# samyak0210/ViNet

Hardware: AMD Instinct MI355X
Metric: clips/sec training (32x224x384 bf16) (higher is better)
Workload: dtype bf16; 1 GPU; ViNet DHF1K training, 32x224x384 bf16, 192 clip(s)/GPU/step, kldiv + fused Adam, 1xMI355X; global_batch=192, local_batch=192, parallelism=dp1

## Files before the change

### include/vinet_hip.h

```cpp
#ifndef VINET_HIP_H
#define VINET_HIP_H

#include <stddef.h>
#include <stdint.h>

#ifdef __cplusplus
extern "C" {
#endif

#define VINET_ABI_VERSION 16

enum { VINET_F32 = 0, VINET_BF16 = 1,
       VINET_F32S = 2 };
enum { VINET_ACT_NONE = 0, VINET_ACT_RELU = 1, VINET_ACT_SIGMOID = 2 };
enum { VINET_CONV_GENERIC = 0, VINET_CONV_STEM = 1 };

typedef struct VinetTensor {
  void* ptr;
  int32_t B, T, H, W, C;
  int32_t ld;
  int64_t sB;
} VinetTensor;

typedef struct VinetAffine {
// ... 115 lines not shown
int vinet_channel_sum(const VinetTensor* x, int32_t dtype, float* workspace, int32_t Cout, float* out,
                      int32_t accumulate, void* stream);

typedef struct VinetPoolDesc {
  int32_t dtype;
  int32_t kT, kH, kW, sT, sH, sW, pT, pH, pW;
} VinetPoolDesc;
int vinet_maxpool3d(const VinetPoolDesc* d, const VinetTensor* x, VinetAffine pre, const VinetTensor* y,
                    uint8_t* argmax, void* stream);
int vinet_maxpool3d_bwd(const VinetPoolDesc* d, const VinetTensor* dy, const uint8_t* argmax, const VinetTensor* dx,
                        int32_t accumulate, void* stream);
int vinet_maxpool3d_kernel_name(const VinetPoolDesc* d, const VinetTensor* x, VinetAffine pre, const VinetTensor* y,
                                const uint8_t* argmax, char* buf, int32_t n);
int vinet_maxpool3d_bwd_kernel_name(const VinetPoolDesc* d, const VinetTensor* dy, const uint8_t* argmax,
                                    const VinetTensor* dx, char* buf, int32_t n);
int vinet_bn_bwd_pool_ok(const VinetPoolDesc* pool, const VinetTensor* z, const VinetTensor* dp, const VinetTensor* dx, int32_t dtype);
int vinet_bn_bwd_reduce_pool(const VinetPoolDesc* pool, const VinetTensor* dp, const uint8_t* argmax, const VinetTensor* gacc,
                             int32_t accumulate, const VinetTensor* z, int32_t dtype, VinetAffine fwd, const float* mean,
                             const float* invstd, float* partials, void* stream);
int vinet_bn_bwd_apply_pool(const VinetPoolDesc* pool, const VinetTensor* dp, const uint8_t* argmax, const VinetTensor* gacc,
                            int32_t accumulate, const VinetTensor* z, int32_t dtype, VinetAffine fwd, const float* mean,
                            const float* invstd, const float* c1, const float* c2, const VinetTensor* dx, void* stream);

int vinet_upsample2x(const VinetTensor* x, const VinetTensor* y, int32_t dtype, void* stream);
int vinet_upsample2x_bwd(const VinetTensor* dy, const VinetTensor* dx, int32_t dtype, int32_t accumulate, void* stream);
int vinet_upsample2x_bwd_relu(const VinetTensor* dy, const VinetTensor* dx, const VinetTensor* xf, int32_t dtype, void* stream);

int vinet_unfold1d(const VinetTensor* x, const VinetTensor* y, int32_t dtype, int32_t stride, int32_t pad, void* stream);

int vinet_loss_fwd(int32_t which, const float* s, const void* gt, int32_t gt_is_f64, int32_t B, int32_t n,
// ... 105 lines not shown
```

### vinet_amd/_lib.py

```python
import ctypes as C
import os

HERE = os.path.dirname(os.path.abspath(__file__))
LIB_PATH = os.environ.get("VINET_LIB") or os.path.join(HERE, "libvinet_hip.so")

F32, BF16 = 0, 1
F32S = 2
ACT_NONE, ACT_RELU, ACT_SIGMOID = 0, 1, 2
CONV_GENERIC, CONV_STEM = 0, 1
ABI_VERSION = 16


class CTensor(C.Structure):
    _fields_ = [("ptr", C.c_void_p), ("B", C.c_int32), ("T", C.c_int32), ("H", C.c_int32), ("W", C.c_int32),
                ("C", C.c_int32), ("ld", C.c_int32), ("sB", C.c_int64)]


class CAffine(C.Structure):
    _fields_ = [("scale", C.c_void_p), ("shift", C.c_void_p), ("relu", C.c_int32)]


class CConvDesc(C.Structure):
    _fields_ = [("dtype", C.c_int32), ("out_dtype", C.c_int32), ("mode", C.c_int32), ("x", CTensor), ("y", CTensor),
                ("oT", C.c_int32), ("oH", C.c_int32), ("oW", C.c_int32),
# ... 60 lines not shown
    "vinet_bn_bwd_reduce": [_PT, _PT, _i32, CAffine, _vp, _vp, _vp, _vp],
    "vinet_conv3d_wgrad_fuses_bn_bwd": [_PW],
    "vinet_conv3d_fuses_dgrad_phases": [_PC],
    "vinet_conv3d_bn_bwd_stats_rows": [_PC],
    "vinet_bn_partials_fold": [_vp, _i32, _i32, _vp, _i32, _vp],
    "vinet_bn_bwd_finalize": [_vp, _i32, _i32, _i32, _f64, _vp, _i32, _vp, _vp, _vp, _vp, _vp, _vp],
    "vinet_bn_bwd_apply": [_PT, _PT, _i32, CAffine, _vp, _vp, _vp, _vp, _PT, _vp],
    "vinet_bn_bwd_apply_split": [_PT, _PT, CAffine, _vp, _vp, _vp, _vp, _PT, _PT, _PT, _vp],
    "vinet_bn_bwd_pool_ok": [_PP, _PT, _PT, _PT, _i32],
    "vinet_bn_bwd_reduce_pool": [_PP, _PT, _vp, _PT, _i32, _PT, _i32, CAffine, _vp, _vp, _vp, _vp],
    "vinet_bn_bwd_apply_pool": [_PP, _PT, _vp, _PT, _i32, _PT, _i32, CAffine, _vp, _vp, _vp, _vp, _PT, _vp],
    "vinet_act_bwd": [_PT, _i32, _PT, _i32, _i32, _PT, _i32, _vp],
    "vinet_channel_sum": [_PT, _i32, _vp, _i32, _vp, _i32, _vp],
    "vinet_maxpool3d": [_PP, _PT, CAffine, _PT, _vp, _vp],
    "vinet_maxpool3d_bwd": [_PP, _PT, _vp, _PT, _i32, _vp],
    "vinet_maxpool3d_kernel_name": [_PP, _PT, CAffine, _PT, _vp, C.c_char_p, _i32],
    "vinet_maxpool3d_bwd_kernel_name": [_PP, _PT, _vp, _PT, C.c_char_p, _i32],
    "vinet_upsample2x": [_PT, _PT, _i32, _vp],
    "vinet_unfold1d": [_PT, _PT, _i32, _i32, _i32, _vp],
    "vinet_upsample2x_bwd": [_PT, _PT, _i32, _i32, _vp],
    "vinet_upsample2x_bwd_relu": [_PT, _PT, _PT, _i32, _vp],
    "vinet_loss_fwd": [_i32, _vp, _vp, _i32, _i32, _i32, _vp, _vp, _vp],
    "vinet_loss_bwd": [_i32, _vp, _vp, _i32, _i32, _i32, _vp, _vp, _f32, _i32, _vp, _vp],
    "vinet_auc_judd_workspace": [_i32, _i32],
    "vinet_auc_judd": [_vp, _i32, _vp, _i32, _i32, _i32, _i32, _vp, C.c_size_t, _vp, _vp, _vp, _vp],
    "vinet_auc_shuffled_workspace": [_i32, _i32, _i32, _f64],
    "vinet_auc_shuffled": [_vp, _i32, _vp, _i32, _vp, _i32, _i64, _i32, _i32, _i32, _f64, _i64, _vp, _vp, _i32, _vp, C.c_size_t,
                           _vp, _vp, _vp, _vp, _vp],
    "vinet_auc_borji_workspace": [_i32, _i32, _i32, _f64],
    "vinet_auc_borji": [_vp, _i32, _vp, _i32, _i32, _i32, _i32, _f64, _i64, _vp, _vp, _i32, _vp, C.c_size_t, _vp, _vp, _vp, _vp],
# ... 104 lines not shown
```

### vinet_amd/csrc/pool.hip

```cpp
#include "pool_gather.h"

struct PoolP { int kT, kH, kW, sT, sH, sW, pT, pH, pW; FastDiv dsT, dsH, dsW; };
static inline PoolP make_poolp(const VinetPoolDesc* d) {
  PoolP p = {d->kT, d->kH, d->kW, d->sT, d->sH, d->sW, d->pT, d->pH, d->pW, make_fastdiv((uint32_t)d->sT), make_fastdiv((uint32_t)d->sH), make_fastdiv((uint32_t)d->sW)};
  return p;
}

template <typename T> VN_DEV float pool_round(float v) { return v; }
template <> VN_DEV float pool_round<bf16_t>(float v) { return bf2f(f2bf(v)); }
template <typename T> VN_DEV float4 pool_pre4(float4 v, const Affine& pre, int c) {
  v = affine4(v, pre, c);
  if (pre.scale) { v.x = pool_round<T>(v.x); v.y = pool_round<T>(v.y); v.z = pool_round<T>(v.z); v.w = pool_round<T>(v.w); }
  return v;
}
template <typename T> VN_DEV float pool_pre(float f, float sc, float sh, const Affine& pre) {
  float v = fmaf(f, sc, sh);
  if (pre.relu) v = fmaxf(v, 0.f);
  if (pre.scale) v = pool_round<T>(v);
  return v;
}
VN_DEV void pool_column(const TView& v, uint32_t col, int& b, int& h, int& w) {
  const uint32_t r1 = fdiv(col, v.dW);
  w = (int)(col - r1 * (uint32_t)v.W);
  const uint32_t r2 = fdiv(r1, v.dH);
// ... 311 lines not shown
      *(unsigned long long*)(argmax + ovox * y.C + c0) = oi;
    }
  }
}


VN_DEV uint32_t pool_code2(uint32_t u) {
  const uint32_t m = ((u >> 15) & 0x00010001u) * 0x7fffu;
  return u ^ (m | 0x80008000u);
}
VN_DEV uint32_t pool_decode2(uint32_t k) {
  const uint32_t m = (((k >> 15) & 0x00010001u) ^ 0x00010001u) * 0x7fffu;
  return k ^ (m | 0x80008000u);
}

__global__ __launch_bounds__(256) void maxpool_fwd8_pk_kernel(PoolP p, TView x, Affine pre, TView y, uint8_t* __restrict__ argmax, long total) {
  const long i = (long)blockIdx.x * blockDim.x + threadIdx.x;
  if (i >= total) return;
  const int G = y.C >> 3;
  const uint32_t vox_u = (uint32_t)(i / G);
  const int g = (int)(i - (long)vox_u * G);
  int b, to, ho, wo;
  decode_vox(y, (long)vox_u, b, to, ho, wo);
  f32x2_v sc2[4], sh2[4];
  const bool aff = pre.scale != nullptr;
#pragma unroll
  for (int e = 0; e < 4; ++e) {
    sc2[e] = aff ? (f32x2_v){pre.scale[g * 8 + 2 * e], pre.scale[g * 8 + 2 * e + 1]} : (f32x2_v){1.f, 1.f};
    sh2[e] = aff ? (f32x2_v){pre.shift[g * 8 + 2 * e], pre.shift[g * 8 + 2 * e + 1]} : (f32x2_v){0.f, 0.f};
  }
  uint32_t best[8];
// ... 13 lines not shown
        uint32_t w4[4] = {q.x, q.y, q.z, q.w};
        const uint32_t ck = last - (uint32_t)((kt * p.kH + kh) * p.kW + kw);
#pragma unroll
        for (int e = 0; e < 4; ++e) {
          if (aff) {
            if (pre.relu) w4[e] = pre_relu_pair(w4[e], sc2[e], sh2[e]);
            else w4[e] = pack2bf(fmaf(__uint_as_float(w4[e] << 16), sc2[e].x, sh2[e].x), fmaf(__uint_as_float(w4[e] & 0xffff0000u), sc2[e].y, sh2[e].y));
          } else if (pre.relu) {
            asm("v_pk_max_i16 %0, %1, 0" : "=v"(w4[e]) : "v"(w4[e]));
          }
          const uint32_t c = pool_code2(w4[e]);
          const uint32_t klo = (c << 16) | ck, khi = (c & 0xffff0000u) | ck;
          best[2 * e] = best[2 * e] > klo ? best[2 * e] : klo;
          best[2 * e + 1] = best[2 * e + 1] > khi ? best[2 * e + 1] : khi;
        }
      }
    }
  }
  uint32_t ov[4];
  unsigned long long bi = 0;
#pragma unroll
  for (int e = 0; e < 8; ++e) {
    const uint32_t k = best[e];
    if (e & 1) ov[e >> 1] |= k & 0xffff0000u; else ov[e >> 1] = k >> 16;
    bi |= (unsigned long long)(last - (k & 0xffu)) << (8 * e);
  }
  uint4 o;
  o.x = pool_decode2(ov[0]); o.y = pool_decode2(ov[1]); o.z = pool_decode2(ov[2]); o.w = pool_decode2(ov[3]);
  *(uint4*)((bf16_t*)y.p + vox_off(y, b, to, ho, wo) + g * 8) = o;
  if (argmax) *(unsigned long long*)(argmax + (long)vox_u * y.C + g * 8) = bi;
}

__global__ __launch_bounds__(512) void maxpool_k3s1_pk_kernel(TView x, Affine pre, TView y, uint8_t* __restrict__ argmax,
                                                              int tilesH, int tilesW) {
  __shared__ __attribute__((aligned(16))) uint16_t P[2][100][64];
  __shared__ __attribute__((aligned(16))) float S[2][64];
  const int tid = threadIdx.x;
  const int oct = tid & 7, pos = tid >> 3;
  const int ph = pos >> 3, pw = pos & 7;
  int bid = blockIdx.x;
  const int ncg = (x.C + 63) >> 6;
  const int cg = bid % ncg; bid /= ncg;
  const int tw = bid % tilesW; bid /= tilesW;
  const int th = bid % tilesH; bid /= tilesH;
  const int b = bid;
// ... 572 lines not shown
                                                 r.tilesH, r.tilesW);) break;
    case POOL_TSLIDE8:
      DISPATCH_T(d->dtype, T, hipLaunchKernelGGL(maxpool_tslide8_kernel<T>, grid, lanes, 0, s, p, xv, a, yv, argmax, r.n);) break;
    case POOL_TSLIDE:
      DISPATCH_T(d->dtype, T, hipLaunchKernelGGL(maxpool_tslide_kernel<T>, grid, lanes, 0, s, p, xv, a, yv, argmax, r.n);) break;
    case POOL_FWD8_PK: hipLaunchKernelGGL(maxpool_fwd8_pk_kernel, grid, lanes, 0, s, p, xv, a, yv, argmax, r.n); break;
    case POOL_FWD8:
      DISPATCH_T(d->dtype, T, hipLaunchKernelGGL(maxpool_fwd8_kernel<T>, grid, lanes, 0, s, p, xv, a, yv, argmax, r.n);) break;
    case POOL_FWD:
      DISPATCH_T(d->dtype, T, hipLaunchKernelGGL(maxpool_fwd_kernel<T>, grid, lanes, 0, s, p, xv, a, yv, argmax, r.n);) break;
    default: break;
  }
  return vn_launch_status(r.name);
}

extern "C" int vinet_maxpool3d_bwd(const VinetPoolDesc* d, const VinetTensor* dy, const uint8_t* argmax,
                                   const VinetTensor* dx, int32_t accumulate, void* stream) {
  if (pool_bwd_args(d, dy, argmax, dx)) return -1;
  const PoolRoute r = pool_bwd_route(d, dy, argmax, dx);
  const PoolP p = make_poolp(d);
  const TView gv = make_view(*dy), xv = make_view(*dx);
  const hipStream_t s = (hipStream_t)stream;
  const dim3 lanes(256), grid(ew_grid(r.n));
  switch (r.kind) {
    case POOL_BWD_K3S1_TW3: hipLaunchKernelGGL(maxpool_bwd_k3s1_tw3_kernel, grid, lanes, 0, s, gv, argmax, xv, accumulate, r.n); break;
    case POOL_BWD_K3S1_TWALK:
      DISPATCH_T(d->dtype, T, hipLaunchKernelGGL(maxpool_bwd_k3s1_twalk_kernel<T>, grid, lanes, 0, s, gv, argmax, xv, accumulate, r.n);) break;
    case POOL_BWD_K3S1:
      DISPATCH_T(d->dtype, T, hipLaunchKernelGGL(maxpool_bwd_k3s1_kernel<T>, grid, lanes, 0, s, gv, argmax, xv, accumulate, r.n);) break;
    case POOL_BWD_K133S2:
// ... 14 lines not shown
```

### vinet_amd/engine.py

```python
import ctypes as C
import itertools
import math
import os
import weakref

import torch

from . import _lib as L

F32, BF16 = L.F32, L.BF16
F32S = L.F32S
TORCH_DT = {F32: torch.float32, BF16: torch.bfloat16}
ESIZE = {F32: 4, BF16: 2}
EG = {F32: 4, BF16: 8}

_DEFAULT_DTYPE = BF16
_WEIGHTS_EPOCH = 0
_UNPACK_TABLES = {}
_SIDE_STREAMS = {}

_CONFIG = dict(
    WGRAD_SIDE_STREAM=True,
    WGRAD_CUS=208,
    WGRAD_CUS_DEC=208,
# ... 10 lines not shown
    BRANCH_STREAMS_BWD_MIN_BATCH=8,
    BRANCH_STREAMS_SWAP=True,
    STEM_FOLD=True,
    JOINT_ENTRY=1,
    BN_BWD_FUSE=1,
    SHARE_SKIP_GRAD=True,
    DEFER_DECODER_WGRAD=1,
    DEFER_DECODER_WGRAD_F32S=0,
    PERSISTENT_DW=1,
    MATERIALIZE_NT=800,
    SPLIT_WGRAD_BF16=1,
    SPLIT_IN_APPLY=1,
    DGRAD_BN_STATS=1,
    UPSAMPLE_BWD_RELU=1,
    POOL_BWD_IN_BN=1,
    PARAM_GRAD_MODE="fused",
    DBG_SPIN_SIDE=0,
    DBG_SPIN_MAIN=0,
    DBG_SPIN_FORK=0,
    ABLATE="",
)
globals().update(_CONFIG)
_ABLATE, _ABLATE_TAGS = set(), []


def configure(**kw):
    global _ABLATE, _ABLATE_TAGS
    old = {}
    for k, v in kw.items():
        K = k.upper()
# ... 140 lines not shown
        n = self.nvox * self.C
        assert n % 4 == 0
        return View(self.buf, self.off, 1, 1, 1, n // 4, 4, 4, n, self.dt)

    def torch5(self):
        return torch.as_strided(self.buf, (self.B, self.T, self.H, self.W, self.C),
                                (self.sB, self.H * self.W * self.ld, self.W * self.ld, self.ld, 1), self.off)

    def same_dims(self, o):
        return (self.B, self.T, self.H, self.W, self.C) == (o.B, o.T, o.H, o.W, o.C)


class Act:
    __slots__ = ("v", "scale", "shift", "relu", "_grad", "grad_ready", "needs_grad", "parent", "pc0", "pt0", "fold",
                 "indep", "ready_of", "grad_marks", "mean", "invstd", "alias_of", "n_readers", "act_out", "grad_masked", "prows", "bn1",
                 "pool_rec")

    def __init__(self, v, scale=None, shift=None, relu=False, needs_grad=False, mean=None, invstd=None):
        self.v, self.scale, self.shift, self.relu = v, scale, shift, relu
        self.mean, self.invstd = mean, invstd
        self._grad, self.grad_ready, self.needs_grad = None, False, needs_grad
        self.parent, self.pc0, self.pt0 = None, 0, 0
        self.fold = None
        self.indep = False
        self.ready_of = None
        self.grad_marks = 0
        self.alias_of = None
        self.n_readers = 0
        self.act_out = 0
        self.grad_masked = -1
        self.prows = None
        self.bn1 = False
        self.pool_rec = None

    @property
    def plain(self):
        return self.scale is None and not self.relu

    def affine(self):
        return L.CAffine(_ptr(self.scale), _ptr(self.shift), 1 if self.relu else 0)

    def sub_chan(self, c0, c1):
        a = Act(self.v.chan(c0, c1), None if self.scale is None else self.scale[c0:c1],
                None if self.shift is None else self.shift[c0:c1], self.relu, self.needs_grad,
                None if self.mean is None else self.mean[c0:c1], None if self.invstd is None else self.invstd[c0:c1])
        a.parent, a.pc0, a.pt0 = self, c0, None
        return a

# ... 314 lines not shown
    g = a.grad_view()
    B, Cc, T, H, W = gt.shape
    sb, sc, st, sh, sw = gt.stride()
    ctx.call("vinet_import_ncdhw", gt.data_ptr(), sb, sc, st, sh, sw, Cc, C.byref(g.ct()), g.dt, ctx.stream)
    a.mark_grad_ready()


def materialize(ctx, a, dst=None, out_dt=None, share_grad=False):
    v = a.v
    alias = dst is None and (out_dt is None or out_dt == v.dt) and v.dt == ctx.dt
    if dst is None:
        dt = ctx.dt if out_dt is None else out_dt
        dst = Act(View.alloc(v.B, v.T, v.H, v.W, v.C, dt, v.device))
    out = dst.v
    assert out.same_dims(v) and dst.plain
    ctx.call("vinet_copy_affine", C.byref(v.ct()), v.dt, a.affine(), C.byref(out.ct()), out.dt, 0, ctx.stream)
    dst.needs_grad = a.needs_grad
    if alias:
        dst.parent, dst.pc0, dst.pt0 = a, 0, None
        dst.alias_of = a
        return dst
    _note_reader(ctx, a)
    if (share_grad and SHARE_SKIP_GRAD and ctx.recording and a.needs_grad and a.parent is None and a._grad is None
            and dst.parent is not None and out.dt == v.dt):
        a.parent, a.pc0, a.pt0 = dst, 0, None
        return dst
    if ctx.recording and a.needs_grad:
        def bwd():
            dg = dst.grad_view()
            tg = a.grad_view()
            ctx.call("vinet_copy_affine", C.byref(dg.ct()), dg.dt, L.CAffine(None, None, 0), C.byref(tg.ct()), tg.dt,
                     1 if a.is_grad_ready() else 0, ctx.stream)
            a.mark_grad_ready()
        ctx.record(bwd)
    return dst


def new_concat(ctx, B, T, H, W, Ctot, pending):
    v = View.alloc(B, T, H, W, Ctot, ctx.dt, ctx.device)
    if pending:
        st = ctx.training
        return Act(v, ctx.f32(Ctot), ctx.f32(Ctot), relu=True, needs_grad=True, mean=ctx.f32(Ctot) if st else None,
                   invstd=ctx.f32(Ctot) if st else None)
    return Act(v, needs_grad=True)



def _phase_taps_1d(I, O, k, s, p):
    out = []
    for r in range(s):
# ... 781 lines not shown
                and dx.same_dims(bx.v) and x.root().grad_marks + 1 == x.root().n_readers)
    part = None
    for ph in phases:
        d = _conv_desc(ctx, L.CONV_GENERIC, dy, dx, ph["Q"], (1, 1, 1), plan.s, ph["r"], ph["ntaps"], ph["taps"], wt, plan.kp(True),
                       L.CAffine(None, None, 0), n_valid, ph["promise"], acc)
        if want_bnb:
            part = _bnb_partials(ctx, d, bx)
        tag, work = _conv_prof(ctx, d, "dgrad", plan, xv, M, es, es, es, len(phases), "+bnb" if part is not None else "")
        ctx.call("vinet_conv3d", C.byref(d), ctx.stream, tag=tag, work=work)
    x.mark_grad_ready()
    if part is not None:
        _register_bnb(ctx, bx, *part)



def maxpool_forward(ctx, x, k, s, p, dst=None):
    xv = x.v
    od = tuple((d + 2 * pp - kk) // ss + 1 for d, kk, ss, pp in zip((xv.T, xv.H, xv.W), k, s, p))
    if dst is None:
        dst = Act(View.alloc(xv.B, od[0], od[1], od[2], xv.C, xv.dt, xv.device))
    out = dst.v
    assert (out.T, out.H, out.W, out.C) == (od[0], od[1], od[2], xv.C) and dst.plain
    pd = L.CPoolDesc(xv.dt, k[0], k[1], k[2], s[0], s[1], s[2], p[0], p[1], p[2])
    rec = ctx.recording and x.needs_grad
    _note_reader(ctx, x)
    am = torch.empty(out.nvox * out.C, dtype=torch.uint8, device=xv.device) if rec else None
    ptag = "maxpool k%dx%dx%d s%dx%dx%d C%d in%dx%dx%dx%d" % (k + s + (xv.C, xv.B, xv.T, xv.H, xv.W))
    es = ESIZE[xv.dt]
    ctx.call("vinet_maxpool3d", C.byref(pd), C.byref(xv.ct()), x.affine(), C.byref(out.ct()), _ptr(am), ctx.stream,
             tag="maxpool_fwd_kernel | " + ptag, work=dict(flops=0.0, bytes=float((xv.nvox + out.nvox) * xv.C * es)))
    dst.needs_grad = x.needs_grad
    if rec:
        def launch(acc):
            dy = dst.grad_view()
            dx = x.grad_view()
            ctx.call("vinet_maxpool3d_bwd", C.byref(pd), C.byref(dy.ct()), am.data_ptr(), C.byref(dx.ct()),
                     acc, ctx.stream, tag="maxpool_bwd_kernel | " + ptag,
                     work=dict(flops=0.0, bytes=float((xv.nvox + out.nvox) * xv.C * es + out.nvox * xv.C)))

        def bwd():
            acc = 1 if x.is_grad_ready() else 0
            if _pool_bwd_defers(ctx, x, pd, k, s, p):
                dy, dx = dst.grad_view(), x.grad_view()
                if dy.dt == dx.dt == BF16 and ctx.lib.vinet_bn_bwd_pool_ok(C.byref(pd), C.byref(xv.ct()), C.byref(dy.ct()),
                                                                          C.byref(dx.ct()), xv.dt):
# ... 143 lines not shown
```

### vinet_amd/model.py

```python
import ctypes as C

import torch
from torch import nn

from . import _lib as L
from . import engine as E
from .model_utils import (BasicConv3d, BNParams2d, ConvParams, Mixed_3b, Mixed_3c, Mixed_4b, Mixed_4c, Mixed_4d,
                          Mixed_4e, Mixed_4f, Mixed_5b, Mixed_5c, SepConv3d, _Block, _Marker)


def _pool_marker(k, s, p):
    return _Marker("maxpool3d", kernel_size=k, stride=s, padding=p)


class BackBoneS3D(_Block):
    _cpad = 4

    def __init__(self):
        super().__init__()
        self.base1 = nn.Sequential(
            SepConv3d(3, 64, kernel_size=7, stride=2, padding=3),
            _pool_marker((1, 3, 3), (1, 2, 2), (0, 1, 1)),
            BasicConv3d(64, 64, kernel_size=1, stride=1),
            SepConv3d(64, 192, kernel_size=3, stride=1, padding=1),
        )
        self.maxp2 = _pool_marker((1, 3, 3), (1, 2, 2), (0, 1, 1))
        self.base2 = nn.Sequential(Mixed_3b(), Mixed_3c())
        self.maxp3 = _pool_marker((3, 3, 3), (2, 2, 2), (1, 1, 1))
        self.base3 = nn.Sequential(Mixed_4b(), Mixed_4c(), Mixed_4d(), Mixed_4e(), Mixed_4f())
        self.maxt4 = _pool_marker((2, 1, 1), (2, 1, 1), (0, 0, 0))
        self.maxp4 = _pool_marker((1, 2, 2), (1, 2, 2), (0, 0, 0))
        self.base4 = nn.Sequential(Mixed_5b(), Mixed_5c())

    def _fwd(self, ctx, x):
        y = self.base1[0]._fwd(ctx, x)
        y = E.maxpool_forward(ctx, y, (1, 3, 3), (1, 2, 2), (0, 1, 1))
        y = self.base1[2]._fwd(ctx, y)
        y3 = self.base1[3]._fwd(ctx, y)
        y = E.maxpool_forward(ctx, y3, (1, 3, 3), (1, 2, 2), (0, 1, 1))
        y2 = self.base2[1]._fwd(ctx, self.base2[0]._fwd(ctx, y))
        y = E.maxpool_forward(ctx, y2, (3, 3, 3), (2, 2, 2), (1, 1, 1))
        for blk in self.base3:
            y = blk._fwd(ctx, y)
        y1 = y
        y = E.maxpool_forward(ctx, y1, (2, 1, 1), (2, 1, 1), (0, 0, 0))
        y = E.maxpool_forward(ctx, y, (1, 2, 2), (1, 2, 2), (0, 0, 0))
        y0 = self.base4[1]._fwd(ctx, self.base4[0]._fwd(ctx, y))
        return [y0, y1, y2, y3]


DECODER_TAILS = {
    32: dict(k5=2, tail=[(32, 32, 2, False), "relu", (32, 1, 1, True)]),
    16: dict(k5=2, tail=[(32, 1, 1, True)]),
    8: dict(k5=1, tail=[(32, 1, 1, True)]),
    48: dict(k5=2, tail=[(32, 32, 3, True), "relu", (32, 1, 1, True)]),
    64: dict(k5=2, tail=[(32, 32, 4, False), "relu", (32, 1, 1, True)]),
}


class _DecoderConvUp(nn.Module):
    _clips = 32
# ... 7 lines not shown
            return [ConvParams(cin, cout, kernel_size=(kt, 3, 3), stride=(kt, 1, 1), padding=(0, 1, 1), bias=False),
                    _Marker("relu"), self.upsampling]

        self.convtsp1 = nn.Sequential(*stage(1024, 832, 1))
        self.convtsp2 = nn.Sequential(*stage(832, 480, 3))
        self.convtsp3 = nn.Sequential(*stage(480, 192, 5))
        tail = []
        for item in spec["tail"]:
            if item == "relu":
                tail.append(_Marker("relu"))
            else:
                cin, cout, kt, bias = item
                tail.append(ConvParams(cin, cout, kernel_size=(kt, 1, 1), stride=(kt, 1, 1), bias=bias))
        self.convtsp4 = nn.Sequential(*stage(192, 64, 5), *stage(64, 32, spec["k5"]), *tail, _Marker("sigmoid"))

    def _conv_relu_up(self, ctx, conv, x, skip=None):
        z = E.conv_forward(ctx, conv.plan(), x, act=L.ACT_RELU)
        zv = z.v
        if skip is None:
            return E.upsample2x_forward(ctx, z)
        sv = skip.v
        assert (sv.H, sv.W, sv.C) == (2 * zv.H, 2 * zv.W, zv.C), "skip connection shape mismatch"
        cat = E.Act(E.View.alloc(zv.B, zv.T + sv.T, sv.H, sv.W, zv.C, ctx.dt, ctx.device), needs_grad=True)
        E.upsample2x_forward(ctx, z, cat.sub_t(0, zv.T))
        E.materialize(ctx, skip, cat.sub_t(zv.T, zv.T + sv.T), share_grad=True)
        return cat

    def _fwd(self, ctx, y0, y1, y2, y3):
        z = self._conv_relu_up(ctx, self.convtsp1[0], y0, y1)
        z = self._conv_relu_up(ctx, self.convtsp2[0], z, y2)
        z = self._conv_relu_up(ctx, self.convtsp3[0], z, y3)
        z = self._conv_relu_up(ctx, self.convtsp4[0], z)
        z = self._conv_relu_up(ctx, self.convtsp4[3], z)
        convs = [m for m in list(self.convtsp4)[6:] if isinstance(m, ConvParams)]
        for conv in convs[:-1]:
            z = E.conv_forward(ctx, conv.plan(), z, act=L.ACT_RELU)
        head = convs[-1]
        npad = E.rup(head.out_channels, E.EG[ctx.dt])
        return E.conv_forward(ctx, head.plan(), z, act=L.ACT_SIGMOID, out_dt=E.F32, n_pad=npad)

    def forward(self, y0, y1, y2, y3):
        body = _MapBody(self, lambda ctx, *a: self._fwd(ctx, *a), n_feature_inputs=4)
        return E.run_root(body, [y0, y1, y2, y3], list(self.parameters()))[0]


class DecoderConvUp(_DecoderConvUp):
# ... 64 lines not shown
                outs.append(None)
        return outs


class VideoSaliencyModel(nn.Module):
    compute_dtype = None

    def __init__(self, transformer_in_channel=32, nhead=4, use_upsample=True, num_hier=3, num_clips=32):
        super().__init__()
        if not use_upsample or num_hier != 3 or num_clips not in DECODER_TAILS:
            raise NotImplementedError("vinet_amd implements use_upsample=True, num_hier=3, num_clips in {8,16,32,48} (+ the build-defined 64)")
        self.backbone = BackBoneS3D()
        self.num_hier = num_hier
        self.decoder = {8: DecoderConvUp8, 16: DecoderConvUp16, 32: DecoderConvUp, 48: DecoderConvUp48, 64: DecoderConvUp64}[num_clips]()

    def _fwd(self, ctx, x):
        y0, y1, y2, y3 = self.backbone._fwd(ctx, x)
        return self.decoder._fwd(ctx, y0, y1, y2, y3)

    def forward(self, x):
        body = _MapBody(self, self._fwd, video=True)
        return E.run_root(body, [x], list(self.parameters()))[0]



SOUNDNET_LAYERS = [(1, 16, 64, 32, 8), (16, 32, 32, 16, 8), (32, 64, 16, 8, 0), (64, 128, 8, 4, 0),
                   (128, 256, 4, 2, 4), (256, 512, 4, 2, 0), (512, 1024, 4, 2, 0)]


class _Conv2dParams(nn.Conv2d):

    def forward(self, x):
        raise RuntimeError("parameters only")
# ... 74 lines not shown
        if os.path.isfile(self.soundnet_checkpoint):
            self.load_soundnet(self.soundnet_checkpoint)
            print("Loaded SoundNet Weights")
        else:
            import sys
            print("SoundNet weights? (%s not found: default init)" % self.soundnet_checkpoint, file=sys.stderr)
        self.maxpool = _Marker("maxpool3d", kernel_size=(4, 1, 1), stride=(2, 1, 2), padding=(0, 0, 0))
        self.bilinear = _BilinearParams(42, 3, 4 * 7 * 12)

    def load_soundnet(self, path="./soundnet8_final.pth"):
        self.audionet.load_state_dict(torch.load(path, map_location="cpu"))

    def _fwd(self, ctx, x, audio):
        from .fusion import bilinear_forward
        a = self.audionet._fwd(ctx, audio)
        y0, y1, y2, y3 = self.visual_model.backbone._fwd(ctx, x)
        y0 = E.maxpool_forward(ctx, y0, (4, 1, 1), (2, 1, 2), (0, 0, 0))
        fused = bilinear_forward(ctx, self.bilinear, y0, a, (4, 7, 12))
        if self.use_transformer:
            from .fusion import transformer_forward
            tok = E.conv_forward(ctx, self.conv_in_1x1.plan(), fused)
            tok = transformer_forward(ctx, self.transformer, tok)
            fused = E.conv_forward(ctx, self.conv_out_1x1.plan(), tok)
        return self.visual_model.decoder._fwd(ctx, fused, y1, y2, y3)

    def forward(self, x, audio):
        body = _MapBody(self, self._fwd, video=True, audio=True)
        return E.run_root(body, [x, audio], list(self.parameters()))[0]


class VideoAudioSaliencyFusionModel(nn.Module):
    compute_dtype = None
    soundnet_checkpoint = "./soundnet8_final.pth"
    unused_parameter_names = ("bilinear.weight", "bilinear.bias")
    graph_capture_refusal = ("a captured step of the token-wise fusion model has never been replayed under test, and a process "
                             "that captured one later crashed inside hipGraph replay (cause not found); run it eagerly")
    N_VIDEO_TOKENS, N_AUDIO_TOKENS = 4 * 7 * 12, 3

    def __init__(self, use_transformer=True, transformer_in_channel=512, num_encoder_layers=3, nhead=4,
# ... 27 lines not shown
            print("SoundNet weights? (%s not found: default init)" % self.soundnet_checkpoint, file=sys.stderr)
        self.maxpool = _Marker("maxpool3d", kernel_size=(4, 1, 1), stride=(2, 1, 2), padding=(0, 0, 0))
        self.bilinear = _BilinearParams(42, 3, 4 * 7 * 12)

    def load_soundnet(self, path="./soundnet8_final.pth"):
        self.audionet.load_state_dict(torch.load(path, map_location="cpu"))

    def _fwd(self, ctx, x, audio):
        from . import fusion
        xv = x.v
        H, W = x.fold if x.fold is not None else (xv.H, xv.W)
        if (xv.T, H, W) != (32, 224, 384):
            raise ValueError("the fusion model runs on 32 x 224 x 384 clips (its 336 position tokens are y0's 4 x 7 x 12 positions, "
                             "model.py:143,180), got %d x %d x %d" % (xv.T, H, W))
        a = self.audionet._fwd(ctx, audio)
        y0, y1, y2, y3 = self.visual_model.backbone._fwd(ctx, x)
        assert (a.v.T, a.v.H, a.v.W) == (self.N_AUDIO_TOKENS, 1, 1), "SoundNet gives %d time steps for this waveform, the model has 3 audio tokens" % a.v.T
        tokens, (vid, aud) = fusion.token_buffer(ctx, xv.B, [(4, 7, 12), (self.N_AUDIO_TOKENS, 1, 1)], self.conv_in_1x1.out_channels)
        E.conv_forward(ctx, self.conv_in_1x1.plan(), y0, dst=vid)
        E.conv_forward(ctx, self.audio_conv_1x1.plan(), a, dst=aud)
        enc = fusion.token_encoder_forward(ctx, self.transformer, tokens)
        fused = fusion.token_split_forward(ctx, enc, self.N_AUDIO_TOKENS, (4, 7, 12))
        return self.visual_model.decoder._fwd(ctx, fused, y1, y2, y3)

    def forward(self, x, audio):
        body = _MapBody(self, self._fwd, video=True, audio=True)
        return E.run_root(body, [x, audio], list(self.parameters()))[0]


class _BilinearParams(nn.Bilinear):
    def forward(self, a, b):
        raise RuntimeError("parameters only")



TRANSFORMER_MAX_HEAD_WIDTH = 96
TOKEN_ENCODER_MAX_HEAD_WIDTH = 128

# ... 71 lines not shown
```

Baseline: 710.0 clips/s.

## Write decoder skip inputs into concat buffers from the maxpool forward pass

The maxpool forward kernel gains a KEEP variant. While it reads each input voxel once, it also stores the voxel (with the affine pre-applied) into the slice of the decoder's concat buffer allocated up front. The decoder then skips the separate copy_affine that used to materialize each skip tensor into the concat, removing one full read and write of three large backbone activations. The cost is extra non-temporal stores inside the pool kernel, shape-prediction logic to preallocate the concat buffers, and a more fragile coupling between backbone and decoder.

Result: faster. 717.9 clips/s (median of 6 runs) (+1.1%).

```diff
diff --git a/include/vinet_hip.h b/include/vinet_hip.h
--- a/include/vinet_hip.h
+++ b/include/vinet_hip.h
@@ -153,6 +153,10 @@
                                 const uint8_t* argmax, char* buf, int32_t n);
 int vinet_maxpool3d_bwd_kernel_name(const VinetPoolDesc* d, const VinetTensor* dy, const uint8_t* argmax,
                                     const VinetTensor* dx, char* buf, int32_t n);
+int vinet_maxpool3d_keep_ok(const VinetPoolDesc* d, const VinetTensor* x, VinetAffine pre, const VinetTensor* y,
+                            const uint8_t* argmax, const VinetTensor* keep);
+int vinet_maxpool3d_keep(const VinetPoolDesc* d, const VinetTensor* x, VinetAffine pre, const VinetTensor* y,
+                         uint8_t* argmax, const VinetTensor* keep, void* stream);
 int vinet_bn_bwd_pool_ok(const VinetPoolDesc* pool, const VinetTensor* z, const VinetTensor* dp, const VinetTensor* dx, int32_t dtype);
 int vinet_bn_bwd_reduce_pool(const VinetPoolDesc* pool, const VinetTensor* dp, const uint8_t* argmax, const VinetTensor* gacc,
                              int32_t accumulate, const VinetTensor* z, int32_t dtype, VinetAffine fwd, const float* mean,
diff --git a/vinet_amd/_lib.py b/vinet_amd/_lib.py
--- a/vinet_amd/_lib.py
+++ b/vinet_amd/_lib.py
@@ -98,6 +98,8 @@
     "vinet_channel_sum": [_PT, _i32, _vp, _i32, _vp, _i32, _vp],
     "vinet_maxpool3d": [_PP, _PT, CAffine, _PT, _vp, _vp],
     "vinet_maxpool3d_bwd": [_PP, _PT, _vp, _PT, _i32, _vp],
+    "vinet_maxpool3d_keep_ok": [_PP, _PT, CAffine, _PT, _vp, _PT],
+    "vinet_maxpool3d_keep": [_PP, _PT, CAffine, _PT, _vp, _PT, _vp],
     "vinet_maxpool3d_kernel_name": [_PP, _PT, CAffine, _PT, _vp, C.c_char_p, _i32],
     "vinet_maxpool3d_bwd_kernel_name": [_PP, _PT, _vp, _PT, C.c_char_p, _i32],
     "vinet_upsample2x": [_PT, _PT, _i32, _vp],
diff --git a/vinet_amd/csrc/pool.hip b/vinet_amd/csrc/pool.hip
--- a/vinet_amd/csrc/pool.hip
+++ b/vinet_amd/csrc/pool.hip
@@ -349,7 +349,9 @@
   return k ^ (m | 0x80008000u);
 }
 
-__global__ __launch_bounds__(256) void maxpool_fwd8_pk_kernel(PoolP p, TView x, Affine pre, TView y, uint8_t* __restrict__ argmax, long total) {
+template <bool KEEP>
+VN_DEV void maxpool_fwd8_pk_lane(const PoolP& p, const TView& x, const Affine& pre, const TView& y, uint8_t* __restrict__ argmax, long total,
+                                 const TView& keep) {
   const long i = (long)blockIdx.x * blockDim.x + threadIdx.x;
   if (i >= total) return;
   const int G = y.C >> 3;
@@ -393,6 +395,8 @@
           best[2 * e] = best[2 * e] > klo ? best[2 * e] : klo;
           best[2 * e + 1] = best[2 * e + 1] > khi ? best[2 * e + 1] : khi;
         }
+        if (KEEP && (unsigned)(kt - p.pT) < (unsigned)p.sT && (unsigned)(kh - p.pH) < (unsigned)p.sH && (unsigned)(kw - p.pW) < (unsigned)p.sW)
+          st16_nt((bf16_t*)keep.p + vox_off(keep, b, t, h, w) + g * 8, make_uint4(w4[0], w4[1], w4[2], w4[3]));
       }
     }
   }
@@ -408,6 +412,13 @@
   o.x = pool_decode2(ov[0]); o.y = pool_decode2(ov[1]); o.z = pool_decode2(ov[2]); o.w = pool_decode2(ov[3]);
   *(uint4*)((bf16_t*)y.p + vox_off(y, b, to, ho, wo) + g * 8) = o;
   if (argmax) *(unsigned long long*)(argmax + (long)vox_u * y.C + g * 8) = bi;
+}
+__global__ __launch_bounds__(256) void maxpool_fwd8_pk_kernel(PoolP p, TView x, Affine pre, TView y, uint8_t* __restrict__ argmax, long total) {
+  maxpool_fwd8_pk_lane<false>(p, x, pre, y, argmax, total, x);
+}
+__global__ __launch_bounds__(256) void maxpool_fwd8_pk_keep_kernel(PoolP p, TView x, Affine pre, TView y, uint8_t* __restrict__ argmax,
+                                                                   long total, TView keep) {
+  maxpool_fwd8_pk_lane<true>(p, x, pre, y, argmax, total, keep);
 }
 
 __global__ __launch_bounds__(512) void maxpool_k3s1_pk_kernel(TView x, Affine pre, TView y, uint8_t* __restrict__ argmax,
@@ -1010,6 +1021,36 @@
   return vn_launch_status(r.name);
 }
 
+static int pool_keep_args(const char* who, const VinetPoolDesc* d, const VinetTensor* x, VinetAffine pre, const VinetTensor* y,
+                          const uint8_t* argmax, const VinetTensor* keep) {
+  if (pool_fwd_args(d, x, pre, y)) return -1;
+  VN_CHECK_ARG(keep, "%s: null argument", who);
+  VN_CHECK_ARG(d->dtype == VINET_BF16, "%s: bf16 only (pool dtype %d)", who, d->dtype);
+  VN_CHECK_ARG(d->sT > 0 && d->sH > 0 && d->sW > 0 && d->pT >= 0 && d->pH >= 0 && d->pW >= 0, "%s: bad stride or padding", who);
+  VN_CHECK_ARG(pool_fwd_route(d, x, y, argmax).kind == POOL_FWD8_PK, "%s: the pool runs on %s, not on maxpool_fwd8_pk_kernel", who,
+               pool_fwd_route(d, x, y, argmax).name);
+  VN_CHECK_ARG(oct_ok(*keep) && same_dims(*keep, *x), "%s: keep is off the 16-byte, 8-channel grid or differs from x in its dims", who);
+  VN_CHECK_ARG(d->kT >= d->pT + d->sT && d->kH >= d->pH + d->sH && d->kW >= d->pW + d->sW,
+               "%s: window %dx%dx%d / s(%d,%d,%d) / p(%d,%d,%d) lacks the taps [p, p + s) that own the input", who, d->kT, d->kH, d->kW,
+               d->sT, d->sH, d->sW, d->pT, d->pH, d->pW);
+  VN_CHECK_ARG((long)y->T * d->sT >= x->T && (long)y->H * d->sH >= x->H && (long)y->W * d->sW >= x->W,
+               "%s: outputs [%d,%d,%d] x strides (%d,%d,%d) do not cover the input [%d,%d,%d]", who, y->T, y->H, y->W, d->sT, d->sH, d->sW,
+               x->T, x->H, x->W);
+  return 0;
+}
+extern "C" int vinet_maxpool3d_keep_ok(const VinetPoolDesc* d, const VinetTensor* x, VinetAffine pre, const VinetTensor* y,
+                                       const uint8_t* argmax, const VinetTensor* keep) {
+  return pool_keep_args("maxpool3d_keep_ok", d, x, pre, y, argmax, keep) == 0 ? 1 : 0;
+}
+extern "C" int vinet_maxpool3d_keep(const VinetPoolDesc* d, const VinetTensor* x, VinetAffine pre, const VinetTensor* y,
+                                    uint8_t* argmax, const VinetTensor* keep, void* stream) {
+  if (pool_keep_args("maxpool3d_keep", d, x, pre, y, argmax, keep)) return -1;
+  const PoolRoute r = pool_fwd_route(d, x, y, argmax);
+  hipLaunchKernelGGL((maxpool_fwd8_pk_keep_kernel), dim3(ew_grid(r.n)), dim3(256), 0, (hipStream_t)stream, make_poolp(d), make_view(*x),
+                     make_affine(pre), make_view(*y), argmax, r.n, make_view(*keep));
+  return vn_launch_status("maxpool_fwd8_pk_keep_kernel");
+}
+
 extern "C" int vinet_maxpool3d_bwd(const VinetPoolDesc* d, const VinetTensor* dy, const uint8_t* argmax,
                                    const VinetTensor* dx, int32_t accumulate, void* stream) {
   if (pool_bwd_args(d, dy, argmax, dx)) return -1;
diff --git a/vinet_amd/engine.py b/vinet_amd/engine.py
--- a/vinet_amd/engine.py
+++ b/vinet_amd/engine.py
@@ -48,6 +48,7 @@
     DGRAD_BN_STATS=1,
     UPSAMPLE_BWD_RELU=1,
     POOL_BWD_IN_BN=1,
+    POOL_KEEPS_SKIP=1,
     PARAM_GRAD_MODE="fused",
     DBG_SPIN_SIDE=0,
     DBG_SPIN_MAIN=0,
@@ -218,7 +219,7 @@
 class Act:
     __slots__ = ("v", "scale", "shift", "relu", "_grad", "grad_ready", "needs_grad", "parent", "pc0", "pt0", "fold",
                  "indep", "ready_of", "grad_marks", "mean", "invstd", "alias_of", "n_readers", "act_out", "grad_masked", "prows", "bn1",
-                 "pool_rec")
+                 "pool_rec", "kept_in")
 
     def __init__(self, v, scale=None, shift=None, relu=False, needs_grad=False, mean=None, invstd=None):
         self.v, self.scale, self.shift, self.relu = v, scale, shift, relu
@@ -236,6 +237,7 @@
         self.prows = None
         self.bn1 = False
         self.pool_rec = None
+        self.kept_in = None
 
     @property
     def plain(self):
@@ -580,7 +582,8 @@
         dst = Act(View.alloc(v.B, v.T, v.H, v.W, v.C, dt, v.device))
     out = dst.v
     assert out.same_dims(v) and dst.plain
-    ctx.call("vinet_copy_affine", C.byref(v.ct()), v.dt, a.affine(), C.byref(out.ct()), out.dt, 0, ctx.stream)
+    if not _same_view(a.kept_in, out):
+        ctx.call("vinet_copy_affine", C.byref(v.ct()), v.dt, a.affine(), C.byref(out.ct()), out.dt, 0, ctx.stream)
     dst.needs_grad = a.needs_grad
     if alias:
         dst.parent, dst.pc0, dst.pt0 = a, 0, None
@@ -600,6 +603,11 @@
             a.mark_grad_ready()
         ctx.record(bwd)
     return dst
+
+
+def _same_view(a, b):
+    return a is not None and a.buf is b.buf and a.dt == b.dt and \
+        (a.off, a.B, a.T, a.H, a.W, a.C, a.ld, a.sB) == (b.off, b.B, b.T, b.H, b.W, b.C, b.ld, b.sB)
 
 
 def new_concat(ctx, B, T, H, W, Ctot, pending):
@@ -1411,7 +1419,12 @@
 
 
 
-def maxpool_forward(ctx, x, k, s, p, dst=None):
+def pool_keeps_skip(ctx):
+    return bool(POOL_KEEPS_SKIP) and ctx.dt == BF16 and getattr(ctx.lib, "vinet_maxpool3d_keep_ok", None) is not None \
+        and hasattr(ctx.lib, "vinet_maxpool3d_keep")
+
+
+def maxpool_forward(ctx, x, k, s, p, dst=None, keep=None):
     xv = x.v
     od = tuple((d + 2 * pp - kk) // ss + 1 for d, kk, ss, pp in zip((xv.T, xv.H, xv.W), k, s, p))
     if dst is None:
@@ -1424,8 +1437,18 @@
     am = torch.empty(out.nvox * out.C, dtype=torch.uint8, device=xv.device) if rec else None
     ptag = "maxpool k%dx%dx%d s%dx%dx%d C%d in%dx%dx%dx%d" % (k + s + (xv.C, xv.B, xv.T, xv.H, xv.W))
     es = ESIZE[xv.dt]
-    ctx.call("vinet_maxpool3d", C.byref(pd), C.byref(xv.ct()), x.affine(), C.byref(out.ct()), _ptr(am), ctx.stream,
-             tag="maxpool_fwd_kernel | " + ptag, work=dict(flops=0.0, bytes=float((xv.nvox + out.nvox) * xv.C * es)))
+    kv = keep.v if keep is not None and pool_keeps_skip(ctx) and keep.plain and keep.v.dt == xv.dt and keep.v.same_dims(xv) else None
+    if kv is not None and not ctx.lib.vinet_maxpool3d_keep_ok(C.byref(pd), C.byref(xv.ct()), x.affine(), C.byref(out.ct()), _ptr(am),
+                                                              C.byref(kv.ct())):
+        kv = None
+    if kv is not None:
+        ctx.call("vinet_maxpool3d_keep", C.byref(pd), C.byref(xv.ct()), x.affine(), C.byref(out.ct()), _ptr(am), C.byref(kv.ct()),
+                 ctx.stream, tag="maxpool_fwd_kernel | " + ptag + " +keep",
+                 work=dict(flops=0.0, bytes=float((2 * xv.nvox + out.nvox) * xv.C * es)))
+        x.kept_in = kv
+    else:
+        ctx.call("vinet_maxpool3d", C.byref(pd), C.byref(xv.ct()), x.affine(), C.byref(out.ct()), _ptr(am), ctx.stream,
+                 tag="maxpool_fwd_kernel | " + ptag, work=dict(flops=0.0, bytes=float((xv.nvox + out.nvox) * xv.C * es)))
     dst.needs_grad = x.needs_grad
     if rec:
         def launch(acc):
diff --git a/vinet_amd/model.py b/vinet_amd/model.py
--- a/vinet_amd/model.py
+++ b/vinet_amd/model.py
@@ -5,7 +5,7 @@
 
 from . import _lib as L
 from . import engine as E
-from .model_utils import (BasicConv3d, BNParams2d, ConvParams, Mixed_3b, Mixed_3c, Mixed_4b, Mixed_4c, Mixed_4d,
+from .model_utils import (MIXED_WIDTHS, BasicConv3d, BNParams2d, ConvParams, Mixed_3b, Mixed_3c, Mixed_4b, Mixed_4c, Mixed_4d,
                           Mixed_4e, Mixed_4f, Mixed_5b, Mixed_5c, SepConv3d, _Block, _Marker)
 
 
@@ -13,6 +13,20 @@
     return _Marker("maxpool3d", kernel_size=k, stride=s, padding=p)
 
 
+def _window_dims(dims, k, s, p):
+    return tuple((d + 2 * pp - kk) // ss + 1 for d, kk, ss, pp in zip(dims, k, s, p))
+
+
+def _sep_dims(sep, dims):
+    for conv in (sep.conv_s, sep.conv_t):
+        dims = _window_dims(dims, conv.kernel_size, conv.stride, conv.padding)
+    return dims
+
+
+POOL_1, POOL_2, POOL_3 = ((1, 3, 3), (1, 2, 2), (0, 1, 1)), ((1, 3, 3), (1, 2, 2), (0, 1, 1)), ((3, 3, 3), (2, 2, 2), (1, 1, 1))
+POOL_T4, POOL_P4 = ((2, 1, 1), (2, 1, 1), (0, 0, 0)), ((1, 2, 2), (1, 2, 2), (0, 0, 0))
+
+
 class BackBoneS3D(_Block):
     _cpad = 4
 
@@ -20,31 +34,41 @@
         super().__init__()
         self.base1 = nn.Sequential(
             SepConv3d(3, 64, kernel_size=7, stride=2, padding=3),
-            _pool_marker((1, 3, 3), (1, 2, 2), (0, 1, 1)),
+            _pool_marker(*POOL_1),
             BasicConv3d(64, 64, kernel_size=1, stride=1),
             SepConv3d(64, 192, kernel_size=3, stride=1, padding=1),
         )
-        self.maxp2 = _pool_marker((1, 3, 3), (1, 2, 2), (0, 1, 1))
+        self.maxp2 = _pool_marker(*POOL_2)
         self.base2 = nn.Sequential(Mixed_3b(), Mixed_3c())
-        self.maxp3 = _pool_marker((3, 3, 3), (2, 2, 2), (1, 1, 1))
+        self.maxp3 = _pool_marker(*POOL_3)
         self.base3 = nn.Sequential(Mixed_4b(), Mixed_4c(), Mixed_4d(), Mixed_4e(), Mixed_4f())
-        self.maxt4 = _pool_marker((2, 1, 1), (2, 1, 1), (0, 0, 0))
-        self.maxp4 = _pool_marker((1, 2, 2), (1, 2, 2), (0, 0, 0))
+        self.maxt4 = _pool_marker(*POOL_T4)
+        self.maxp4 = _pool_marker(*POOL_P4)
         self.base4 = nn.Sequential(Mixed_5b(), Mixed_5c())
 
-    def _fwd(self, ctx, x):
+    def feature_dims(self, T, H, W):
+        d = _window_dims(_sep_dims(self.base1[0], (T, H, W)), *POOL_1)
+        d3 = _sep_dims(self.base1[3], d)
+        d2 = _window_dims(d3, *POOL_2)
+        d1 = _window_dims(d2, *POOL_3)
+        d0 = _window_dims(_window_dims(d1, *POOL_T4), *POOL_P4)
+        widths = [sum(MIXED_WIDTHS[n][i] for i in (1, 3, 5, 6)) for n in ("5c", "4f", "3c")]
+        return [d0 + (widths[0],), d1 + (widths[1],), d2 + (widths[2],), d3 + (self.base1[3].conv_t.out_channels,)]
+
+    def _fwd(self, ctx, x, keep=None):
+        k1, k2, k3 = keep if keep is not None else (None, None, None)
         y = self.base1[0]._fwd(ctx, x)
-        y = E.maxpool_forward(ctx, y, (1, 3, 3), (1, 2, 2), (0, 1, 1))
+        y = E.maxpool_forward(ctx, y, *POOL_1)
         y = self.base1[2]._fwd(ctx, y)
         y3 = self.base1[3]._fwd(ctx, y)
-        y = E.maxpool_forward(ctx, y3, (1, 3, 3), (1, 2, 2), (0, 1, 1))
+        y = E.maxpool_forward(ctx, y3, *POOL_2, keep=k3)
         y2 = self.base2[1]._fwd(ctx, self.base2[0]._fwd(ctx, y))
-        y = E.maxpool_forward(ctx, y2, (3, 3, 3), (2, 2, 2), (1, 1, 1))
+        y = E.maxpool_forward(ctx, y2, *POOL_3, keep=k2)
         for blk in self.base3:
             y = blk._fwd(ctx, y)
         y1 = y
-        y = E.maxpool_forward(ctx, y1, (2, 1, 1), (2, 1, 1), (0, 0, 0))
-        y = E.maxpool_forward(ctx, y, (1, 2, 2), (1, 2, 2), (0, 0, 0))
+        y = E.maxpool_forward(ctx, y1, *POOL_T4, keep=k1)
+        y = E.maxpool_forward(ctx, y, *POOL_P4)
         y0 = self.base4[1]._fwd(ctx, self.base4[0]._fwd(ctx, y))
         return [y0, y1, y2, y3]
 
@@ -82,22 +106,36 @@
                 tail.append(ConvParams(cin, cout, kernel_size=(kt, 1, 1), stride=(kt, 1, 1), bias=bias))
         self.convtsp4 = nn.Sequential(*stage(192, 64, 5), *stage(64, 32, spec["k5"]), *tail, _Marker("sigmoid"))
 
-    def _conv_relu_up(self, ctx, conv, x, skip=None):
+    def _conv_relu_up(self, ctx, conv, x, skip=None, cat=None):
         z = E.conv_forward(ctx, conv.plan(), x, act=L.ACT_RELU)
         zv = z.v
         if skip is None:
             return E.upsample2x_forward(ctx, z)
         sv = skip.v
         assert (sv.H, sv.W, sv.C) == (2 * zv.H, 2 * zv.W, zv.C), "skip connection shape mismatch"
-        cat = E.Act(E.View.alloc(zv.B, zv.T + sv.T, sv.H, sv.W, zv.C, ctx.dt, ctx.device), needs_grad=True)
+        if cat is None or (cat.v.B, cat.v.T, cat.v.H, cat.v.W, cat.v.C, cat.v.dt) != (zv.B, zv.T + sv.T, sv.H, sv.W, zv.C, ctx.dt):
+            cat = E.Act(E.View.alloc(zv.B, zv.T + sv.T, sv.H, sv.W, zv.C, ctx.dt, ctx.device), needs_grad=True)
         E.upsample2x_forward(ctx, z, cat.sub_t(0, zv.T))
         E.materialize(ctx, skip, cat.sub_t(zv.T, zv.T + sv.T), share_grad=True)
         return cat
 
-    def _fwd(self, ctx, y0, y1, y2, y3):
-        z = self._conv_relu_up(ctx, self.convtsp1[0], y0, y1)
-        z = self._conv_relu_up(ctx, self.convtsp2[0], z, y2)
-        z = self._conv_relu_up(ctx, self.convtsp3[0], z, y3)
+    def skip_concats(self, ctx, B, d0, skips):
+        cats, keep, d = [], [], tuple(d0)
+        for conv, (sT, sH, sW, sC) in zip((self.convtsp1[0], self.convtsp2[0], self.convtsp3[0]), skips):
+            zT, zH, zW = conv.plan().out_dims(*d)
+            if zT < 1 or (sH, sW, sC) != (2 * zH, 2 * zW, conv.out_channels):
+                return None
+            cat = E.Act(E.View.alloc(B, zT + sT, sH, sW, sC, ctx.dt, ctx.device), needs_grad=True)
+            cats.append(cat)
+            keep.append(E.Act(cat.v.tslice(zT, zT + sT)))
+            d = (zT + sT, sH, sW)
+        return cats, tuple(keep)
+
+    def _fwd(self, ctx, y0, y1, y2, y3, cats=None):
+        c1, c2, c3 = cats if cats is not None else (None, None, None)
+        z = self._conv_relu_up(ctx, self.convtsp1[0], y0, y1, c1)
+        z = self._conv_relu_up(ctx, self.convtsp2[0], z, y2, c2)
+        z = self._conv_relu_up(ctx, self.convtsp3[0], z, y3, c3)
         z = self._conv_relu_up(ctx, self.convtsp4[0], z)
         z = self._conv_relu_up(ctx, self.convtsp4[3], z)
         convs = [m for m in list(self.convtsp4)[6:] if isinstance(m, ConvParams)]
@@ -192,9 +230,21 @@
         self.num_hier = num_hier
         self.decoder = {8: DecoderConvUp8, 16: DecoderConvUp16, 32: DecoderConvUp, 48: DecoderConvUp48, 64: DecoderConvUp64}[num_clips]()
 
+    def _skip_concats(self, ctx, x, d0=None):
+        if not E.pool_keeps_skip(ctx):
+            return None, None
+        xv = x.v
+        H, W = x.fold if x.fold is not None else (xv.H, xv.W)
+        f = self.backbone.feature_dims(xv.T, H, W)
+        if min(min(d) for d in f) < 1:
+            return None, None
+        got = self.decoder.skip_concats(ctx, xv.B, f[0][:3] if d0 is None else d0, f[1:])
+        return got if got is not None else (None, None)
+
     def _fwd(self, ctx, x):
-        y0, y1, y2, y3 = self.backbone._fwd(ctx, x)
-        return self.decoder._fwd(ctx, y0, y1, y2, y3)
+        cats, keep = self._skip_concats(ctx, x)
+        y0, y1, y2, y3 = self.backbone._fwd(ctx, x, keep)
+        return self.decoder._fwd(ctx, y0, y1, y2, y3, cats)
 
     def forward(self, x):
         body = _MapBody(self, self._fwd, video=True)
@@ -299,7 +349,8 @@
     def _fwd(self, ctx, x, audio):
         from .fusion import bilinear_forward
         a = self.audionet._fwd(ctx, audio)
-        y0, y1, y2, y3 = self.visual_model.backbone._fwd(ctx, x)
+        cats, keep = self.visual_model._skip_concats(ctx, x, (4, 7, 12))
+        y0, y1, y2, y3 = self.visual_model.backbone._fwd(ctx, x, keep)
         y0 = E.maxpool_forward(ctx, y0, (4, 1, 1), (2, 1, 2), (0, 0, 0))
         fused = bilinear_forward(ctx, self.bilinear, y0, a, (4, 7, 12))
         if self.use_transformer:
@@ -307,7 +358,7 @@
             tok = E.conv_forward(ctx, self.conv_in_1x1.plan(), fused)
             tok = transformer_forward(ctx, self.transformer, tok)
             fused = E.conv_forward(ctx, self.conv_out_1x1.plan(), tok)
-        return self.visual_model.decoder._fwd(ctx, fused, y1, y2, y3)
+        return self.visual_model.decoder._fwd(ctx, fused, y1, y2, y3, cats)
 
     def forward(self, x, audio):
         body = _MapBody(self, self._fwd, video=True, audio=True)
@@ -365,14 +416,15 @@
             raise ValueError("the fusion model runs on 32 x 224 x 384 clips (its 336 position tokens are y0's 4 x 7 x 12 positions, "
                              "model.py:143,180), got %d x %d x %d" % (xv.T, H, W))
         a = self.audionet._fwd(ctx, audio)
-        y0, y1, y2, y3 = self.visual_model.backbone._fwd(ctx, x)
+        cats, keep = self.visual_model._skip_concats(ctx, x, (4, 7, 12))
+        y0, y1, y2, y3 = self.visual_model.backbone._fwd(ctx, x, keep)
         assert (a.v.T, a.v.H, a.v.W) == (self.N_AUDIO_TOKENS, 1, 1), "SoundNet gives %d time steps for this waveform, the model has 3 audio tokens" % a.v.T
         tokens, (vid, aud) = fusion.token_buffer(ctx, xv.B, [(4, 7, 12), (self.N_AUDIO_TOKENS, 1, 1)], self.conv_in_1x1.out_channels)
         E.conv_forward(ctx, self.conv_in_1x1.plan(), y0, dst=vid)
         E.conv_forward(ctx, self.audio_conv_1x1.plan(), a, dst=aud)
         enc = fusion.token_encoder_forward(ctx, self.transformer, tokens)
         fused = fusion.token_split_forward(ctx, enc, self.N_AUDIO_TOKENS, (4, 7, 12))
-        return self.visual_model.decoder._fwd(ctx, fused, y1, y2, y3)
+        return self.visual_model.decoder._fwd(ctx, fused, y1, y2, y3, cats)
 
     def forward(self, x, audio):
         body = _MapBody(self, self._fwd, video=True, audio=True)
```
